# facebookresearch/metamorph

Hardware: AMD Instinct MI355X
Metric: train tokens/sec (LLaMA-3-8B + SigLIP-SO400M, seq2048, 256 img toks), whole job (higher is better)
Workload: dtype bf16

## Files before the change

include/mm355.h:

```cpp
#ifndef MM355_H
#define MM355_H

#include <stddef.h>
#include <stdint.h>

#ifdef __cplusplus
extern "C" {
#endif

#define MM355_VERSION 100

#define MM355_OK            0
#define MM355_EINVAL       -1
#define MM355_EUNSUPPORTED -2
#define MM355_ELAUNCH      -3

typedef uint16_t mm355_bf16;

int mm355_version(void);
const char* mm355_strerror(int code);

#define MM355_GEMM_BIAS        1u
#define MM355_GEMM_GELU_ERF    2u
#define MM355_GEMM_GELU_TANH   4u
// ... 17 lines not shown
int64_t mm355_gemm_splitk_swiglu_ws_floats(int64_t M, int64_t I, int64_t K);
int mm355_gemm_splitk_swiglu_bf16(const mm355_bf16* X, int64_t ldx, const mm355_bf16* Wgu, int64_t ldw, mm355_bf16* act, int64_t ld_act,
                                  int64_t M, int64_t I, int64_t K, float* workspace, int64_t workspace_floats, void* stream);
int mm355_gemm_splitk_rope_append_bf16(const mm355_bf16* X, int64_t ldx, const mm355_bf16* Wqkv, int64_t ldw, mm355_bf16* qkv, int64_t ld_qkv,
                                       int64_t M, int64_t Hq, int64_t Hkv, int64_t d, int64_t K, const mm355_bf16* cos_t,
                                       const mm355_bf16* sin_t, const int32_t* positions, mm355_bf16* k_cache, mm355_bf16* v_cache,
                                       int64_t ld_kv, int64_t batch_stride_kv, float* workspace, int64_t workspace_floats, void* stream);

int mm355_gemm_swiglu_bf16(const mm355_bf16* X, int64_t ldx, const mm355_bf16* Wgu, int64_t ldw, mm355_bf16* gu, int64_t ld_gu,
                           mm355_bf16* act, int64_t ld_act, int64_t M, int64_t I, int64_t K, void* stream);

int mm355_gemm_rope_bf16(const mm355_bf16* X, int64_t ldx, const mm355_bf16* Wqkv, int64_t ldw, mm355_bf16* qkv, int64_t ld_qkv,
                         const mm355_bf16* cos_t, const mm355_bf16* sin_t, const int32_t* pos_offset,
                         int64_t M, int64_t N, int64_t K, int64_t L, int64_t n_rot, void* stream);

int mm355_gemm_swiglu_bwd_bf16(const mm355_bf16* dY, int64_t ldy, const mm355_bf16* WdT, int64_t ldw, const mm355_bf16* gu, int64_t ld_gu,
                               mm355_bf16* dgu, int64_t ld_dgu, mm355_bf16* actT, mm355_bf16* dguT, int64_t ldT,
                               int64_t M, int64_t I, int64_t K, void* stream);

int mm355_gemm_pair_bf16(const mm355_bf16* A0, int64_t lda0, const mm355_bf16* B0, int64_t ldb0, void* C0, int64_t ldc0,
                         int64_t M0, int64_t N0, int64_t K0, uint32_t flags0,
                         const mm355_bf16* A1, int64_t lda1, const mm355_bf16* B1, int64_t ldb1, void* C1, int64_t ldc1,
                         int64_t M1, int64_t N1, int64_t K1, uint32_t flags1, void* stream);

int mm355_transpose_bf16(const mm355_bf16* in, int64_t ld_in, int64_t rows, int64_t cols,
                         mm355_bf16* out, int64_t ld_out, void* stream);

int mm355_colsum_bf16(const mm355_bf16* dY, int64_t ld, int64_t M, int64_t N, float* db_f32, void* stream);

int mm355_rmsnorm_fwd(const mm355_bf16* x, const mm355_bf16* w, mm355_bf16* y, int64_t M, int64_t h,
                      float eps, void* stream);
int mm355_rmsnorm_fwd_rstd(const mm355_bf16* x, const mm355_bf16* w, mm355_bf16* y, float* rstd_out, int64_t M, int64_t h,
                           float eps, void* stream);
int mm355_rmsnorm_apply_t(const mm355_bf16* x, const mm355_bf16* w, const float* rstd, int64_t M, int64_t h,
                          mm355_bf16* out_t, int64_t ld_out, void* stream);
int mm355_rmsnorm_bwd(const mm355_bf16* dy, const mm355_bf16* x, const mm355_bf16* w,
                      const mm355_bf16* dres, mm355_bf16* dx, float* dw_f32, float* workspace,
                      int64_t M, int64_t h, float eps, void* stream);
int64_t mm355_rmsnorm_bwd_ws_floats(int64_t M, int64_t h);
int mm355_rmsnorm_bwd_wgrad(const mm355_bf16* dy, const mm355_bf16* x, const mm355_bf16* w, const mm355_bf16* dres,
                            mm355_bf16* dx, mm355_bf16* w_grad, int accumulate, float* workspace,
                            int64_t M, int64_t h, float eps, void* stream);

int mm355_layernorm_fwd(const mm355_bf16* x, const mm355_bf16* w, const mm355_bf16* b, mm355_bf16* y,
                        int64_t M, int64_t h, float eps, void* stream);
int64_t mm355_layernorm_bwd_ws_floats(int64_t M, int64_t h);
// ... 178 lines not shown
                     int64_t n_seg, mm355_bf16* dembed, int64_t h, int accumulate, void* stream);

int mm355_im2col_patch(const void* images, int images_are_f32, int64_t N, int64_t H, int64_t W, int64_t p,
                       mm355_bf16* out, int64_t Kp, void* stream);
int mm355_bilinear_l2norm(const mm355_bf16* in, mm355_bf16* out, int64_t N, int64_t side_in, int64_t side_out,
                          int64_t C, int normalize, void* stream);
int mm355_bilinear_l2norm_bwd(const mm355_bf16* in, const mm355_bf16* d_out, float* d_in_f32, int64_t N, int64_t side_in,
                              int64_t side_out, int64_t C, int normalize, void* stream);

int mm355_cosine_loss(const mm355_bf16* pred_raw, const mm355_bf16* target, int64_t R, int64_t C, int normalize,
                      float* cos_sum, mm355_bf16* dpred, float* row_ws, void* stream);

int mm355_mean_abs_loss(const mm355_bf16* pred, const mm355_bf16* target, int64_t R, int64_t C, float* abs_sum,
                        mm355_bf16* dpred, float* row_ws, void* stream);
int mm355_soft_ce_loss(const mm355_bf16* pred_raw, const mm355_bf16* target, int64_t R, int64_t C, int normalize,
                       float temperature, float* loss_sum, mm355_bf16* dpred, float* row_ws, void* stream);
int mm355_softmax_rows(const mm355_bf16* x, mm355_bf16* y, int64_t R, int64_t C, float temperature, void* stream);
int mm355_softmax_rows_bwd(const mm355_bf16* y, const mm355_bf16* dy, mm355_bf16* dx, int64_t R, int64_t C,
                           float temperature, void* stream);

int mm355_adamw_shard(float* p32, float* m, float* v, const mm355_bf16* g, mm355_bf16* p_out, int64_t n,
                      float lr, float beta1, float beta2, float eps, float weight_decay,
                      float bias_corr1, float bias_corr2, const float* grad_scale_dev, void* stream);
#define MM355_SUMSQ_PARTIALS 2048
int mm355_sumsq_bf16(const mm355_bf16* x, int64_t n, float* out, float* partials, void* stream);
int mm355_clip_coef(const float* sumsq, float max_norm, float pre_scale, float* coef, void* stream);

#ifdef __cplusplus
}
#endif
#endif
```

metamorph_amd/csrc/elementwise.hip:

```cpp
#include "mm355_common.h"
#include <algorithm>

namespace {

constexpr int NT = 256;
constexpr int MAX_GRID = 256 * 16;

inline unsigned grid_for(int64_t work_items) {
    int64_t g = (work_items + NT - 1) / NT;
    if (g > MAX_GRID) g = MAX_GRID;
    if (g < 1) g = 1;
    return (unsigned)g;
}

__global__ void rope_table_kernel(uint16_t* __restrict__ cos_o, uint16_t* __restrict__ sin_o, int L, int d, float theta) {
    const int half = d >> 1;
    for (int64_t i = blockIdx.x * (int64_t)NT + threadIdx.x; i < (int64_t)L * half; i += (int64_t)gridDim.x * NT) {
        const int l = (int)(i / half), j = (int)(i % half);
        const float inv = 1.0f / powf(theta, (float)(2 * j) / (float)d);
        const float ang = (float)l * inv;
        const uint16_t c = f2bf(cosf(ang)), s = f2bf(sinf(ang));
        cos_o[(int64_t)l * d + j] = c; cos_o[(int64_t)l * d + half + j] = c;
        sin_o[(int64_t)l * d + j] = s; sin_o[(int64_t)l * d + half + j] = s;
    }
}

__global__ void rope_table_freq_kernel(uint16_t* __restrict__ cos_o, uint16_t* __restrict__ sin_o, int L, int d,
                                       const float* __restrict__ inv_freq, float scaling) {
    const int half = d >> 1;
// ... 150 lines not shown
template <typename TX>
__global__ __launch_bounds__(NT) void axpy_kernel(uint16_t* __restrict__ y, const TX* __restrict__ x, int64_t n, const float* __restrict__ s_dev,
                                                  float s_host, int accumulate) {
    const float s = (s_dev ? *s_dev : 1.0f) * s_host;
    for (int64_t i = blockIdx.x * (int64_t)NT + threadIdx.x; i < n; i += (int64_t)gridDim.x * NT) {
        float xv;
        if constexpr (sizeof(TX) == 2) xv = bf2f(x[i]); else xv = x[i];
        float r = s * xv;
        if (accumulate) r += bf2f(y[i]);
        y[i] = f2bf(r);
    }
}
__global__ __launch_bounds__(NT) void cast2d_kernel(const float* __restrict__ in, int64_t ld_in, uint16_t* __restrict__ out, int64_t ld_out, int64_t rows, int cols) {
    const int cv = cols >> 3;
    const int64_t total = rows * cv;
    for (int64_t i = blockIdx.x * (int64_t)NT + threadIdx.x; i < total; i += (int64_t)gridDim.x * NT) {
        const int64_t r = i / cv; const int c = (int)(i % cv) * 8;
        const f32x4 a = *(const f32x4*)(in + r * ld_in + c), b = *(const f32x4*)(in + r * ld_in + c + 4);
        const float f[8] = {a.x, a.y, a.z, a.w, b.x, b.y, b.z, b.w};
        *(u32x4*)(out + r * ld_out + c) = pack8(f);
    }
}

__global__ __launch_bounds__(NT) void adamw_kernel(float* __restrict__ p32, float* __restrict__ m, float* __restrict__ v, const uint16_t* __restrict__ g,
                                                   uint16_t* __restrict__ pout, int64_t n, float lr, float b1, float b2, float eps, float wd,
                                                   float bc1, float bc2, const float* __restrict__ gs_dev) {
    const float gs = gs_dev ? *gs_dev : 1.0f;
    const float inv_sqrt_bc2 = rsqrtf(bc2);
    const float step = lr / bc1;
    for (int64_t i = blockIdx.x * (int64_t)NT + threadIdx.x; i < n; i += (int64_t)gridDim.x * NT) {
        const float gr = bf2f(g[i]) * gs;
        float p = p32[i] * (1.0f - lr * wd);
        const float mi = m[i] * b1 + (1.0f - b1) * gr;
        const float vi = v[i] * b2 + (1.0f - b2) * gr * gr;
        const float denom = sqrtf(vi) * inv_sqrt_bc2 + eps;
        p -= step * (mi / denom);
        m[i] = mi; v[i] = vi; p32[i] = p;
        pout[i] = f2bf(p);
    }
}
__global__ __launch_bounds__(NT) void sumsq_kernel(const uint16_t* __restrict__ x, int64_t n, float* __restrict__ partials) {
    __shared__ float red[NT / 64];
    float s = 0.f;
    const int64_t nv = n >> 3;
    for (int64_t v = blockIdx.x * (int64_t)NT + threadIdx.x; v < nv; v += (int64_t)gridDim.x * NT) {
        float f[8];
        unpack8(*(const u32x4*)(x + v * 8), f);
#pragma unroll
        for (int e = 0; e < 8; ++e) s += f[e] * f[e];
    }
    if (blockIdx.x == 0 && threadIdx.x < (n & 7)) { const float f = bf2f(x[(nv << 3) + threadIdx.x]); s += f * f; }
    s = block_sum<NT>(s, red);
    if (threadIdx.x == 0) partials[blockIdx.x] = s;
}
__global__ __launch_bounds__(NT) void sumsq_finish_kernel(const float* __restrict__ partials, int count, float* __restrict__ out) {
    __shared__ float red[NT / 64];
    float s = 0.f;
    for (int i = threadIdx.x; i < count; i += NT) s += partials[i];
    s = block_sum<NT>(s, red);
// ... 158 lines not shown
    if (!x || n <= 0 || !mm_aligned16(x)) return MM355_EINVAL;
    LAUNCH(scale_kernel, grid_for(n / 8 + 1), x, n, s_dev, s_host);
}
extern "C" int mm355_axpy_bf16(mm355_bf16* y, const mm355_bf16* x, int64_t n, const float* s_dev, float s_host, int accumulate, void* stream) {
    (void)hipGetLastError();
    if (!x || !y || n <= 0) return MM355_EINVAL;
    LAUNCH(axpy_kernel<uint16_t>, grid_for(n), y, x, n, s_dev, s_host, accumulate);
}
extern "C" int mm355_axpy_f32_to_bf16(mm355_bf16* y, const float* x, int64_t n, float s_host, int accumulate, void* stream) {
    (void)hipGetLastError();
    if (!x || !y || n <= 0) return MM355_EINVAL;
    LAUNCH(axpy_kernel<float>, grid_for(n), y, x, n, (const float*)nullptr, s_host, accumulate);
}
extern "C" int mm355_axpy_f32_to_bf16_dev(mm355_bf16* y, const float* x, int64_t n, const float* s_dev, float s_host, int accumulate, void* stream) {
    (void)hipGetLastError();
    if (!x || !y || n <= 0) return MM355_EINVAL;
    LAUNCH(axpy_kernel<float>, grid_for(n), y, x, n, s_dev, s_host, accumulate);
}
extern "C" int mm355_cast_f32_bf16_2d(const float* in, int64_t ld_in, mm355_bf16* out, int64_t ld_out, int64_t rows, int64_t cols, void* stream) {
    (void)hipGetLastError();
    if (!in || !out || rows <= 0 || cols <= 0 || (cols & 7) || (ld_in & 3) || (ld_out & 7)) return MM355_EINVAL;
    LAUNCH(cast2d_kernel, grid_for(rows * (cols / 8)), in, ld_in, out, ld_out, rows, (int)cols);
}
extern "C" int mm355_adamw_shard(float* p32, float* m, float* v, const mm355_bf16* g, mm355_bf16* p_out, int64_t n, float lr, float beta1,
                                 float beta2, float eps, float weight_decay, float bias_corr1, float bias_corr2, const float* grad_scale_dev,
                                 void* stream) {
    (void)hipGetLastError();
    if (!p32 || !m || !v || !g || !p_out || n <= 0 || bias_corr1 <= 0.f || bias_corr2 <= 0.f) return MM355_EINVAL;
    LAUNCH(adamw_kernel, grid_for(n), p32, m, v, g, p_out, n, lr, beta1, beta2, eps, weight_decay, bias_corr1, bias_corr2, grad_scale_dev);
}
extern "C" int mm355_sumsq_bf16(const mm355_bf16* x, int64_t n, float* out, float* partials, void* stream) {
    (void)hipGetLastError();
    if (!x || !out || !partials || n <= 0 || !mm_aligned16(x)) return MM355_EINVAL;
    const int blocks = (int)std::min<int64_t>((n / 8 + NT) / NT, MM355_SUMSQ_PARTIALS);
    hipLaunchKernelGGL(sumsq_kernel, dim3(blocks), dim3(NT), 0, (hipStream_t)stream, x, n, partials);
    hipLaunchKernelGGL(sumsq_finish_kernel, dim3(1), dim3(NT), 0, (hipStream_t)stream, (const float*)partials, blocks, out);
    return mm_launch_status();
}
extern "C" int mm355_clip_coef(const float* sumsq, float max_norm, float pre_scale, float* coef, void* stream) {
    (void)hipGetLastError();
    if (!sumsq || !coef) return MM355_EINVAL;
    hipLaunchKernelGGL(clip_coef_kernel, dim3(1), dim3(1), 0, (hipStream_t)stream, sumsq, max_norm, pre_scale, coef);
    return mm_launch_status();
}
extern "C" int mm355_im2col_patch(const void* images, int images_are_f32, int64_t N, int64_t H, int64_t W, int64_t p, mm355_bf16* out, int64_t Kp,
                                  void* stream) {
    (void)hipGetLastError();
    if (!images || !out || N <= 0 || H < p || W < p || p <= 0 || Kp < 3 * p * p) return MM355_EINVAL;
    const int64_t total = N * (H / p) * (W / p) * Kp;
    if (images_are_f32) LAUNCH(im2col_kernel<float>, grid_for(total), (const float*)images, (int)N, (int)H, (int)W, (int)p, out, (int)Kp);
    LAUNCH(im2col_kernel<uint16_t>, grid_for(total), (const uint16_t*)images, (int)N, (int)H, (int)W, (int)p, out, (int)Kp);
}
// ... 25 lines not shown
```

metamorph_amd/csrc/gemm_bf16.hip:

```cpp
#include "gemm_common.h"
#include "splitk.h"
#include <type_traits>
#include <cstdlib>

namespace {

MM_DEV void gemm_epilogue_swiglu(f32x4 (&acc)[8][4], const GemmArgs& a, unsigned char* smem, int m0, int tn, int wm, int wn, int wave, int lane) {
    constexpr int TN = 64;
    const int fr = lane & 15, fq = lane >> 4;
    const int M = a.M, I = (int)a.res_mod;
    float* stg = (float*)smem + wave * (16 * TN);
    const int row_l = lane >> 2, k4 = lane & 3;
    uint16_t* gu = (uint16_t*)a.C;
    uint16_t* act = (uint16_t*)a.res;
    const int ch0 = tn * 128 + wn * 32;
#pragma unroll
    for (int i = 0; i < 8; ++i) {
        __builtin_amdgcn_fence(__ATOMIC_RELEASE, "wavefront");
        __builtin_amdgcn_wave_barrier();
#pragma unroll
        for (int j = 0; j < 4; ++j)
#pragma unroll
            for (int r = 0; r < 4; ++r) stg[(fq * 4 + r) * TN + j * 16 + fr] = acc[i][j][r];
        __builtin_amdgcn_fence(__ATOMIC_RELEASE, "wavefront");
// ... 638 lines not shown
}

template <int ABL = 0>
__global__ __launch_bounds__(512) void gemm_pp_kernel(GemmArgs a) {
    extern __shared__ __attribute__((aligned(16))) unsigned char smem[];
#ifdef MM355_PP_PERSIST
    const int total = a.ntm * a.ntn;
    for (int bid = blockIdx.x; bid < total; bid += gridDim.x) {
        gemm_pp_tile<ABL>(a, bid, smem);
        __syncthreads();
    }
#else
    gemm_pp_tile<ABL>(a, blockIdx.x, smem);
#endif
}

__global__ __launch_bounds__(512) void gemm_pp_pair_kernel(GemmArgs a0, GemmArgs a1, int n0) {
    extern __shared__ __attribute__((aligned(16))) unsigned char smem[];
    const int bid = blockIdx.x;
    if (bid < n0) gemm_pp_tile(a0, bid, smem);
    else gemm_pp_tile(a1, bid - n0, smem);
}

template <int BM, int BN, int WM, int WN, bool GLDS, int PIPE>
int launch_gemm(GemmArgs a, hipStream_t s);

constexpr int PP_LDS = 2 * (256 + 256) * 128;

int64_t pp_prepare(GemmArgs& a) {
    a.ntm = (a.M + 255) / 256;
    a.ntn = (a.N + 255) / 256;
    a.gm = 4;
    return (int64_t)a.ntm * a.ntn;
}

template <int ABL = 0>
int launch_gemm_pp_t(GemmArgs a, hipStream_t s) {
    static std::atomic<uint64_t> lds_ok{0};
    if (mm_ensure_dynamic_lds((const void*)gemm_pp_kernel<ABL>, PP_LDS, lds_ok) != MM355_OK) return MM355_ELAUNCH;
    const int64_t total = pp_prepare(a);
    if (total <= 0 || total > 0x7fffffff) return MM355_EINVAL;
#ifdef MM355_PP_PERSIST
    hipLaunchKernelGGL((gemm_pp_kernel<ABL>), dim3((unsigned)std::min<int64_t>(total, MM355_PP_PERSIST)), dim3(512), PP_LDS, s, a);
#else
    hipLaunchKernelGGL((gemm_pp_kernel<ABL>), dim3((unsigned)total), dim3(512), PP_LDS, s, a);
#endif
    return mm_launch_status();
}

int launch_gemm_pp_pair(GemmArgs a0, GemmArgs a1, hipStream_t s) {
    static std::atomic<uint64_t> lds_ok{0};
    if (mm_ensure_dynamic_lds((const void*)gemm_pp_pair_kernel, PP_LDS, lds_ok) != MM355_OK) return MM355_ELAUNCH;
    const int64_t n0 = pp_prepare(a0), n1 = pp_prepare(a1);
    if (n0 <= 0 || n1 <= 0 || n0 + n1 > 0x7fffffff) return MM355_EINVAL;
    hipLaunchKernelGGL(gemm_pp_pair_kernel, dim3((unsigned)(n0 + n1)), dim3(512), PP_LDS, s, a0, a1, (int)n0);
    return mm_launch_status();
}

bool pp_eligible(const GemmArgs& a) {
    if (a.K < 128 || (a.K & 127)) return false;
    const int64_t ea = (256 * a.lda + a.K) * 2;
    const int64_t eb = (256 * a.ldb + a.K) * 2;
    return ea < 0x7fffffffLL && eb < 0x7fffffffLL;
}

int launch_gemm_pp(GemmArgs a, hipStream_t s) {
    if (!pp_eligible(a)) return launch_gemm<256, 256, 2, 4, true, 1>(a, s);
    return launch_gemm_pp_t(a, s);
}

template <int BM, int BN, int WM, int WN, bool GLDS, int PIPE = 0>
int launch_gemm(GemmArgs a, hipStream_t s) {
    constexpr int STAGE = (BM + BN) * 128;
    constexpr int LDS = 2 * STAGE;
    auto kern = gemm_nt_kernel<BM, BN, WM, WN, GLDS, PIPE>;
    static std::atomic<uint64_t> lds_ok{0};
    if (mm_ensure_dynamic_lds((const void*)kern, LDS, lds_ok) != MM355_OK) return MM355_ELAUNCH;
    a.ntm = (a.M + BM - 1) / BM;
// ... 422 lines not shown
    if (!dma_ok && variant != 1) return MM355_EUNSUPPORTED;
    switch (variant) {
        case 1: return launch_gemm<128, 128, 2, 2, false>(a, s);
        case 2: return launch_gemm<128, 128, 2, 2, true>(a, s);
        case 7: return launch_gemm<256, 256, 2, 4, true, 1>(a, s);
        case 9: return launch_gemm<64, 128, 1, 4, true>(a, s);
        case 11: return launch_gemm_pp(a, s);
#ifdef MM355_ABLATIONS
        case 91: return launch_gemm_pp_t<1>(a, s);
        case 92: return launch_gemm_pp_t<2>(a, s);
        case 93: return launch_gemm_pp_t<3>(a, s);
#endif
        default: return MM355_EUNSUPPORTED;
    }
}

namespace {
int pair_problem(GemmArgs& a, const mm355_bf16* A, int64_t lda, const mm355_bf16* B, int64_t ldb, void* C, int64_t ldc,
                 int64_t M, int64_t N, int64_t K, uint32_t flags) {
    if (!A || !B || !C || M <= 0 || N <= 0 || K <= 0) return MM355_EINVAL;
    if ((K & 7) || (lda & 7) || (ldb & 7) || !mm_aligned16(A) || !mm_aligned16(B) || !mm_aligned16(C)) return MM355_EINVAL;
    if (M > 0x7fffffff || N > 0x7fffffff || K > 0x7fffffff) return MM355_EINVAL;
    if (flags & ~(MM355_GEMM_ACCUMULATE | MM355_GEMM_OUT_F32)) return MM355_EINVAL;
    a.A = A; a.B = B; a.C = C; a.bias = nullptr; a.res = nullptr;
    a.lda = lda; a.ldb = ldb; a.ldc = ldc; a.ldr = 0; a.res_mod = 0;
    a.M = (int)M; a.N = (int)N; a.K = (int)K; a.flags = flags; a.ntm = a.ntn = 0;
    return pp_eligible(a) ? MM355_OK : MM355_EUNSUPPORTED;
}
}

extern "C" int mm355_gemm_pair_bf16(const mm355_bf16* A0, int64_t lda0, const mm355_bf16* B0, int64_t ldb0, void* C0, int64_t ldc0,
                                    int64_t M0, int64_t N0, int64_t K0, uint32_t flags0,
                                    const mm355_bf16* A1, int64_t lda1, const mm355_bf16* B1, int64_t ldb1, void* C1, int64_t ldc1,
                                    int64_t M1, int64_t N1, int64_t K1, uint32_t flags1, void* stream) {
    (void)hipGetLastError();
    GemmArgs a0, a1;
    int rc = pair_problem(a0, A0, lda0, B0, ldb0, C0, ldc0, M0, N0, K0, flags0);
    if (rc != MM355_OK) return rc;
    rc = pair_problem(a1, A1, lda1, B1, ldb1, C1, ldc1, M1, N1, K1, flags1);
    if (rc != MM355_OK) return rc;
    return launch_gemm_pp_pair(a0, a1, (hipStream_t)stream);
}

extern "C" int mm355_transpose_bf16(const mm355_bf16* in, int64_t ld_in, int64_t rows, int64_t cols, mm355_bf16* out,
                                    int64_t ld_out, void* stream) {
    (void)hipGetLastError();
    if (!in || !out || rows <= 0 || cols <= 0 || (ld_in & 7) || !mm_aligned16(in) || !mm_aligned16(out)) return MM355_EINVAL;
    if (ld_out < rows || rows > 0x7fffffff || cols > 0x7fffffff) return MM355_EINVAL;
    dim3 grid((unsigned)((cols + 63) / 64), (unsigned)((rows + 63) / 64));
    hipLaunchKernelGGL(transpose_kernel, grid, dim3(256), 0, (hipStream_t)stream, in, ld_in, (int)rows, (int)cols, out, ld_out);
    return mm_launch_status();
}

extern "C" int mm355_gemm_swiglu_bf16(const mm355_bf16* X, int64_t ldx, const mm355_bf16* Wgu, int64_t ldw, mm355_bf16* gu, int64_t ld_gu,
                                      mm355_bf16* act, int64_t ld_act, int64_t M, int64_t I, int64_t K, void* stream) {
    (void)hipGetLastError();
    if (!X || !Wgu || !gu || !act || M <= 0 || I <= 0 || K <= 0) return MM355_EINVAL;
    if ((ldx & 7) || (ldw & 7) || (ld_gu & 7) || (ld_act & 7) || !mm_aligned16(X) || !mm_aligned16(Wgu) || !mm_aligned16(gu) || !mm_aligned16(act))
        return MM355_EINVAL;
    if (M > 0x7fffffff || I > 0x3fffffff || K > 0x7fffffff) return MM355_EINVAL;
    if ((I & 127) || K < 128 || (K & 127) || (2 * I * ldw + K) * 2 >= 0x7fffffffLL || (256 * ldx + K) * 2 >= 0x7fffffffLL) return MM355_EUNSUPPORTED;
    GemmArgs a = {};
    a.A = X; a.B = Wgu; a.C = gu; a.bias = nullptr; a.res = act;
    a.lda = ldx; a.ldb = ldw; a.ldc = ld_gu; a.ldr = ld_act; a.res_mod = I;
// ... 65 lines not shown
```

metamorph_amd/functional.py:

```python
from __future__ import annotations

import os

import numpy as np
import torch
from torch.autograd import Function

from . import ops

BF16 = torch.bfloat16
VARIANTS = {"fuse_swiglu": True, "fuse_rope": True, "fuse_swiglu_bwd": True, "decode_graph": True, "decode_fused": True,
            "wt_cache": False,
            "decode_fold_rows": 4,
            "prefill_splitk": True,
            "decode_wide_fused": True, "decode_wide_gu_gemv": True,
            "prefill_fused": True,
            "w8_gemm": True,
            "extend_pass": True, "extend_min_rows": 3}


def set_variant(name, value):
    if name not in VARIANTS:
        raise KeyError(f"unknown variant {name!r}: {sorted(VARIANTS)}")
    old, VARIANTS[name] = VARIANTS[name], (int(value) if isinstance(VARIANTS[name], int) and not isinstance(VARIANTS[name], bool) else bool(value))
    return old


_CUS = 256



def _adjacent(ts):
    t0 = ts[0]
    ptr = t0.data_ptr()
    st = t0.untyped_storage()
    total = sum(t.numel() * t.element_size() for t in ts)
    if ptr - st.data_ptr() + total > st.nbytes():
        return False
    for t in ts:
        if (not t.is_contiguous() or t.data_ptr() != ptr or t.shape[1:] != t0.shape[1:] or t.dtype != t0.dtype
                or t.untyped_storage().data_ptr() != st.data_ptr()):
# ... 150 lines not shown
def transposed_weight(w, sources=None):
    if sources is None or not VARIANTS["wt_cache"]:
        return transpose_padded(w)
    key = (w.untyped_storage().data_ptr(), w.storage_offset(), tuple(w.shape), tuple(w.stride()))
    stamp = (param_generation(),) + tuple(p._version for p in sources)
    hit = _WT_CACHE.get(key)
    if hit is not None and hit[0] == stamp:
        return hit[1]
    if _WT_CACHE and next(iter(_WT_CACHE.values()))[0][0] != stamp[0]:
        _WT_CACHE.clear()
    wt = transpose_padded(w)
    _WT_CACHE[key] = (stamp, wt)
    return wt


def drop_transposed_weights():
    _WT_CACHE.clear()


def _pairable(a0, b0, a1, b1):
    t0 = -(-a0.shape[0] // 256) * -(-b0.shape[0] // 256)
    t1 = -(-a1.shape[0] // 256) * -(-b1.shape[0] // 256)
    return min(t0, t1) >= 200 and t0 % 8 == 0 and ops.gemm_pair_supported(a0, b0, a1, b1)


def input_grad_gemm(dy2d, w, out=None, residual=None):
    return ops.gemm(dy2d, transposed_weight(w), out=out, residual=residual)



class LayerMeta:

    def __init__(self, B, L, Hq, Hkv, d, I, eps, cos, sin, seqlens, recompute=False, pos_offset=None, c2p=None, p2c=None):
        self.B, self.L, self.Hq, self.Hkv, self.d, self.I, self.eps = B, L, Hq, Hkv, d, I, eps
        self.cos, self.sin, self.seqlens = cos, sin, seqlens
        self.pos_offset = pos_offset
        self.c2p, self.p2c = c2p, p2c
        self.prompt_pass = False
        self.scale = d ** -0.5
        self.recompute = recompute


PROMPT_GU_SPLITK_ROWS = 64


def decoder_layer_forward(x, layer, m: LayerMeta):
# ... 127 lines not shown
                do = torch.empty((dx2.shape[0], woT.shape[0]), device=dev, dtype=BF16)
                ops.gemm_pair(a0, b0, buf, acc, dx2, woT, do, False)
            else:
                do = ops.gemm(dx2, woT)
                ops.gemm(a0, b0, out=buf, accumulate=acc)
            del a0, b0, woT
            commit_grad(att.o_proj.weight, buf)
        if do is None:
            do = input_grad_gemm(dx2, att.o_proj.weight)
        dqkv = torch.empty_like(qkv)
        fuse_rope = VARIANTS["fuse_rope"] and ops.attn_bwd_rope_supported(m.d)
        o_att = o
        if m.p2c is not None:
            o_att, do = ops.rows_gather(o, m.p2c), ops.rows_gather(do, m.p2c)
        ops.attn_bwd(qkv[:, :nq], qkv[:, nq:nq + nk], qkv[:, nq + nk:], o_att, do, lse, m.B, m.L, m.Hq, m.Hkv, m.d,
                     m.scale, True, m.seqlens, dqkv[:, :nq], dqkv[:, nq:nq + nk], dqkv[:, nq + nk:],
                     rope=(m.cos, m.sin, m.pos_offset) if fuse_rope else None)
        del do, o_att
        if not fuse_rope:
            ops.rope_qk_(dqkv, m.B, m.L, m.Hq, m.Hkv, m.d, m.cos, m.sin, inverse=True, pos_offset=m.pos_offset)
        if m.c2p is not None:
            dqkv = ops.rows_gather(dqkv, m.c2p)
        wqkv = fused_weight(qkv_params)
        dn1 = ops.gemm(dqkv, transposed_weight(wqkv, sources=qkv_params))
        if any(p.requires_grad for p in qkv_params):
            fb, acc, bufs = fused_grad_target(qkv_params)
            n1T = ops.rmsnorm_apply_t(x, layer.input_layernorm.weight, rstd1, _padded_rows(x.shape[0], long_k=True))
            if held is not None:
                a1, b1 = _dw_operands(dqkv, None, xT=n1T)
                if ops.gemm_pair_supported(held[0], held[1], a1, b1):
                    ops.gemm_pair(held[0], held[1], held[2], held[3], a1, b1, fb, bool(acc))
                else:
                    ops.gemm(held[0], held[1], out=held[2], accumulate=held[3])
                    ops.gemm(a1, b1, out=fb, accumulate=bool(acc))
                held = None
                del a1, b1
            else:
                weight_grad_gemm(dqkv, None, fb, bool(acc), xT=n1T)
            commit_fused_grad(qkv_params, fb, acc, bufs)
            del n1T
        del dqkv
        dx = _rmsnorm_backward(dn1, x, layer.input_layernorm.weight, m.eps, dx2)
        if _LAYER_GRAD_HOOK is not None:
            _LAYER_GRAD_HOOK(layer)
        return (dx, None, None) + (None,) * (len(ctx.needs_input_grad) - 3)


def decoder_layer(x, layer, meta):
    params_ready(layer)
    ws = [p for p in layer.parameters()]
    if torch.is_grad_enabled() and (x.requires_grad or any(p.requires_grad for p in ws)):
        return DecoderLayerFn.apply(x, layer, meta, *ws)
    return decoder_layer_forward(x, layer, meta)[0]



class RmsNormFn(Function):
    @staticmethod
    def forward(ctx, x, w, eps):
        ctx.save_for_backward(x, w)
        ctx.eps = eps
        return ops.rmsnorm_fwd(x, w.data if isinstance(w, torch.nn.Parameter) else w, eps)

# ... 1052 lines not shown
```

metamorph_amd/ops.py:

```python
from __future__ import annotations

import os

import torch

from . import lib as _lib

BF16 = torch.bfloat16

GEMM_BIAS, GEMM_GELU_ERF, GEMM_GELU_TANH, GEMM_RESIDUAL, GEMM_ACCUMULATE, GEMM_OUT_F32 = 1, 2, 4, 8, 16, 32
GELU_ERF, GELU_TANH = 0, 1


def _L():
    return _lib.load()


def _stream():
    return torch.cuda.current_stream().cuda_stream


def _chk_dev(*ts):
    for t in ts:
        if t is not None and not t.is_cuda:
# ... 128 lines not shown
def gemm_pair_supported(a0, b0, a1, b1):
    return (a0.shape[1] == b0.shape[1] and a1.shape[1] == b1.shape[1]
            and gemm_pp_operands_ok(a0.shape[1], a0, b0) and gemm_pp_operands_ok(a1.shape[1], a1, b1))


def gemm_pair(a0, b0, out0, acc0, a1, b1, out1, acc1):
    _chk_dev(a0, b0, out0, a1, b1, out1)
    probs = []
    for a, b, out, acc in ((a0, b0, out0, acc0), (a1, b1, out1, acc1)):
        assert a.dtype == BF16 and b.dtype == BF16
        pa, M, K, lda = _rows2d(a)
        pb, N, Kb, ldb = _rows2d(b)
        assert K == Kb, (a.shape, b.shape)
        po, Mo, No, ldc = _rows2d(out)
        assert (Mo, No) == (M, N), (out.shape, M, N)
        assert out.dtype in (BF16, torch.float32)
        flags = (GEMM_ACCUMULATE if acc else 0) | (GEMM_OUT_F32 if out.dtype == torch.float32 else 0)
        probs += [pa, lda, pb, ldb, po, ldc, M, N, K, flags]
    _lib.check(_L().mm355_gemm_pair_bf16(*probs, _stream()),
               f"mm355_gemm_pair_bf16 {tuple(a0.shape)}x{tuple(b0.shape)} + {tuple(a1.shape)}x{tuple(b1.shape)}")
    return out0, out1


def gemm_pp_operands_ok(K, *mats):
    return K >= 128 and K % 128 == 0 and all(256 * m.stride(0) * 2 < 2 ** 31 - 2 ** 20 for m in mats)


def gemv_supported(x, w):
    _, M, K, ldx = _rows2d(x)
    _, N, _, ldw = _rows2d(w)
    if M > 32 or (M > 16 and not gemv_rows32_units((N + 3) // 4)):
        return False
    return M <= 4 or ((N - 1) * ldw * 2 + K * 2 < 0xf0000000 and (M - 1) * ldx * 2 + K * 2 < 0xf0000000)


def gemv_rows32_units(units):
    return (units + 3) // 4 > 1280


def gemv(x, w, out=None, bias=None, residual=None, gelu=None):
    _chk_dev(x, w, out, bias, residual)
    px, M, K, ldx = _rows2d(x)
    pw, N, Kw, ldw = _rows2d(w)
    assert K == Kw and x.dtype == BF16 and w.dtype == BF16
    if out is None:
        out = torch.empty((M, N), device=x.device, dtype=BF16)
# ... 905 lines not shown
def bilinear_l2norm(feat, side_in, side_out, normalize):
    _chk_dev(feat)
    assert feat.is_contiguous()
    N, P, C = feat.shape
    assert P == side_in * side_in
    out = torch.empty((N, side_out * side_out, C), device=feat.device, dtype=BF16)
    _lib.check(_L().mm355_bilinear_l2norm(feat.data_ptr(), out.data_ptr(), N, side_in, side_out, C, int(normalize), _stream()), "mm355_bilinear_l2norm")
    return out


def bilinear_l2norm_bwd(x, dy, side_in, side_out, normalize):
    _chk_dev(x, dy)
    assert x.is_contiguous() and dy.is_contiguous()
    N, _, C = x.shape
    acc = torch.zeros(x.shape, device=x.device, dtype=torch.float32)
    _lib.check(_L().mm355_bilinear_l2norm_bwd(x.data_ptr(), dy.data_ptr(), acc.data_ptr(), N, side_in, side_out, C, int(bool(normalize)),
                                              _stream()), "mm355_bilinear_l2norm_bwd")
    out = torch.empty_like(x)
    cast_f32_to_bf16_2d(acc.view(-1, C), out.view(-1, C))
    return out



def adamw_shard_(p32, m, v, g, p_out, lr, beta1, beta2, eps, wd, step, grad_scale_dev=None):
    _chk_dev(p32, m, v, g, p_out)
    n = p32.numel()
    assert m.numel() == n and v.numel() == n and g.numel() == n and p_out.numel() == n
    bc1 = 1.0 - beta1 ** step
    bc2 = 1.0 - beta2 ** step
    _lib.check(_L().mm355_adamw_shard(p32.data_ptr(), m.data_ptr(), v.data_ptr(), g.data_ptr(), p_out.data_ptr(), n, lr, beta1, beta2,
                                      eps, wd, bc1, bc2, _p(grad_scale_dev), _stream()), "mm355_adamw_shard")


SUMSQ_PARTIALS = 2048
_sumsq_partials = {}


def sumsq_(x, out_f32, partials=None):
    _chk_dev(x, out_f32)
    assert x.is_contiguous()
    if partials is None:
        key = (x.device, _stream())
        partials = _sumsq_partials.get(key)
        if partials is None:
            partials = _sumsq_partials[key] = torch.empty(SUMSQ_PARTIALS, dtype=torch.float32, device=x.device)
    assert partials.dtype == torch.float32 and partials.numel() >= SUMSQ_PARTIALS and partials.device == x.device
    _lib.check(_L().mm355_sumsq_bf16(x.data_ptr(), x.numel(), out_f32.data_ptr(), partials.data_ptr(), _stream()), "mm355_sumsq_bf16")
    return out_f32


def clip_coef(sumsq_f32, max_norm, pre_scale, out_f32):
    _chk_dev(sumsq_f32, out_f32)
    _lib.check(_L().mm355_clip_coef(sumsq_f32.data_ptr(), max_norm, pre_scale, out_f32.data_ptr(), _stream()), "mm355_clip_coef")
    return out_f32
# ... 1 lines not shown
```

Before: 26610.

## Group QKV input-grad and weight-grad GEMMs into one launch; vectorize AdamW

```diff
diff --git a/include/mm355.h b/include/mm355.h
--- a/include/mm355.h
+++ b/include/mm355.h
@@ -63,6 +63,17 @@
                          int64_t M0, int64_t N0, int64_t K0, uint32_t flags0,
                          const mm355_bf16* A1, int64_t lda1, const mm355_bf16* B1, int64_t ldb1, void* C1, int64_t ldc1,
                          int64_t M1, int64_t N1, int64_t K1, uint32_t flags1, void* stream);
+
+#define MM355_GEMM_GROUP_MAX 4
+typedef struct mm355_gemm_problem {
+    const mm355_bf16* A; int64_t lda;
+    const mm355_bf16* B; int64_t ldb;
+    void* C; int64_t ldc;
+    const mm355_bf16* residual; int64_t ldr;
+    int64_t M, N, K;
+    uint32_t flags;
+} mm355_gemm_problem;
+int mm355_gemm_group_bf16(const mm355_gemm_problem* problems, int count, void* stream);
 
 int mm355_transpose_bf16(const mm355_bf16* in, int64_t ld_in, int64_t rows, int64_t cols,
                          mm355_bf16* out, int64_t ld_out, void* stream);
@@ -287,6 +298,9 @@
 int mm355_adamw_shard(float* p32, float* m, float* v, const mm355_bf16* g, mm355_bf16* p_out, int64_t n,
                       float lr, float beta1, float beta2, float eps, float weight_decay,
                       float bias_corr1, float bias_corr2, const float* grad_scale_dev, void* stream);
+int mm355_adamw_shard_opt(float* p32, float* m, float* v, const mm355_bf16* g, mm355_bf16* p_out, int64_t n,
+                          float lr, float beta1, float beta2, float eps, float weight_decay,
+                          float bias_corr1, float bias_corr2, const float* grad_scale_dev, int kernel, int grid, void* stream);
 #define MM355_SUMSQ_PARTIALS 2048
 int mm355_sumsq_bf16(const mm355_bf16* x, int64_t n, float* out, float* partials, void* stream);
 int mm355_clip_coef(const float* sumsq, float max_norm, float pre_scale, float* coef, void* stream);
diff --git a/metamorph_amd/csrc/elementwise.hip b/metamorph_amd/csrc/elementwise.hip
--- a/metamorph_amd/csrc/elementwise.hip
+++ b/metamorph_amd/csrc/elementwise.hip
@@ -5,6 +5,7 @@
 
 constexpr int NT = 256;
 constexpr int MAX_GRID = 256 * 16;
+constexpr int ADAMW8_GRID = 256 * 8;
 
 inline unsigned grid_for(int64_t work_items) {
     int64_t g = (work_items + NT - 1) / NT;
@@ -201,6 +202,14 @@
     }
 }
 
+MM_DEV void adamw_elem(float& p, float& mi, float& vi, const float gr, const float lr, const float b1, const float b2, const float eps, const float wd,
+                       const float inv_sqrt_bc2, const float step) {
+    p = p * (1.0f - lr * wd);
+    mi = mi * b1 + (1.0f - b1) * gr;
+    vi = vi * b2 + (1.0f - b2) * gr * gr;
+    const float denom = sqrtf(vi) * inv_sqrt_bc2 + eps;
+    p -= step * (mi / denom);
+}
 __global__ __launch_bounds__(NT) void adamw_kernel(float* __restrict__ p32, float* __restrict__ m, float* __restrict__ v, const uint16_t* __restrict__ g,
                                                    uint16_t* __restrict__ pout, int64_t n, float lr, float b1, float b2, float eps, float wd,
                                                    float bc1, float bc2, const float* __restrict__ gs_dev) {
@@ -209,11 +218,40 @@
     const float step = lr / bc1;
     for (int64_t i = blockIdx.x * (int64_t)NT + threadIdx.x; i < n; i += (int64_t)gridDim.x * NT) {
         const float gr = bf2f(g[i]) * gs;
-        float p = p32[i] * (1.0f - lr * wd);
-        const float mi = m[i] * b1 + (1.0f - b1) * gr;
-        const float vi = v[i] * b2 + (1.0f - b2) * gr * gr;
-        const float denom = sqrtf(vi) * inv_sqrt_bc2 + eps;
-        p -= step * (mi / denom);
+        float p = p32[i], mi = m[i], vi = v[i];
+        adamw_elem(p, mi, vi, gr, lr, b1, b2, eps, wd, inv_sqrt_bc2, step);
+        m[i] = mi; v[i] = vi; p32[i] = p;
+        pout[i] = f2bf(p);
+    }
+}
+__global__ __launch_bounds__(NT) void adamw8_kernel(float* __restrict__ p32, float* __restrict__ m, float* __restrict__ v, const uint16_t* __restrict__ g,
+                                                    uint16_t* __restrict__ pout, int64_t n, float lr, float b1, float b2, float eps, float wd,
+                                                    float bc1, float bc2, const float* __restrict__ gs_dev) {
+    const float gs = gs_dev ? *gs_dev : 1.0f;
+    const float inv_sqrt_bc2 = rsqrtf(bc2);
+    const float step = lr / bc1;
+    const int64_t nv = n >> 3;
+    for (int64_t i = blockIdx.x * (int64_t)NT + threadIdx.x; i < nv; i += (int64_t)gridDim.x * NT) {
+        const int64_t e0 = i << 3;
+        const f32x4 pa = *(const f32x4*)(p32 + e0), pb = *(const f32x4*)(p32 + e0 + 4);
+        const f32x4 ma = *(const f32x4*)(m + e0), mb = *(const f32x4*)(m + e0 + 4);
+        const f32x4 va = *(const f32x4*)(v + e0), vb = *(const f32x4*)(v + e0 + 4);
+        float p[8] = {pa.x, pa.y, pa.z, pa.w, pb.x, pb.y, pb.z, pb.w};
+        float mi[8] = {ma.x, ma.y, ma.z, ma.w, mb.x, mb.y, mb.z, mb.w};
+        float vi[8] = {va.x, va.y, va.z, va.w, vb.x, vb.y, vb.z, vb.w};
+        float gr[8];
+        unpack8(*(const u32x4*)(g + e0), gr);
+#pragma unroll
+        for (int e = 0; e < 8; ++e) adamw_elem(p[e], mi[e], vi[e], gr[e] * gs, lr, b1, b2, eps, wd, inv_sqrt_bc2, step);
+        *(f32x4*)(m + e0) = f32x4{mi[0], mi[1], mi[2], mi[3]}; *(f32x4*)(m + e0 + 4) = f32x4{mi[4], mi[5], mi[6], mi[7]};
+        *(f32x4*)(v + e0) = f32x4{vi[0], vi[1], vi[2], vi[3]}; *(f32x4*)(v + e0 + 4) = f32x4{vi[4], vi[5], vi[6], vi[7]};
+        *(f32x4*)(p32 + e0) = f32x4{p[0], p[1], p[2], p[3]}; *(f32x4*)(p32 + e0 + 4) = f32x4{p[4], p[5], p[6], p[7]};
+        *(u32x4*)(pout + e0) = pack8(p);
+    }
+    if (blockIdx.x == 0 && threadIdx.x < (n & 7)) {
+        const int64_t i = (nv << 3) + threadIdx.x;
+        float p = p32[i], mi = m[i], vi = v[i];
+        adamw_elem(p, mi, vi, bf2f(g[i]) * gs, lr, b1, b2, eps, wd, inv_sqrt_bc2, step);
         m[i] = mi; v[i] = vi; p32[i] = p;
         pout[i] = f2bf(p);
     }
@@ -418,12 +456,26 @@
     if (!in || !out || rows <= 0 || cols <= 0 || (cols & 7) || (ld_in & 3) || (ld_out & 7)) return MM355_EINVAL;
     LAUNCH(cast2d_kernel, grid_for(rows * (cols / 8)), in, ld_in, out, ld_out, rows, (int)cols);
 }
+extern "C" int mm355_adamw_shard_opt(float* p32, float* m, float* v, const mm355_bf16* g, mm355_bf16* p_out, int64_t n, float lr, float beta1,
+                                     float beta2, float eps, float weight_decay, float bias_corr1, float bias_corr2, const float* grad_scale_dev,
+                                     int kernel, int grid, void* stream) {
+    (void)hipGetLastError();
+    if (!p32 || !m || !v || !g || !p_out || n <= 0 || bias_corr1 <= 0.f || bias_corr2 <= 0.f) return MM355_EINVAL;
+    if (kernel < 0 || kernel > 2 || grid < 0 || grid > 65536) return MM355_EINVAL;
+    const bool aligned = mm_aligned16(p32) && mm_aligned16(m) && mm_aligned16(v) && mm_aligned16(g) && mm_aligned16(p_out);
+    if (kernel == 2 && !aligned) return MM355_EINVAL;
+    if (kernel == 1 || !aligned) {
+        LAUNCH(adamw_kernel, grid ? (unsigned)grid : grid_for(n), p32, m, v, g, p_out, n, lr, beta1, beta2, eps, weight_decay, bias_corr1, bias_corr2,
+               grad_scale_dev);
+    }
+    unsigned blocks = grid ? (unsigned)grid : (unsigned)std::min<int64_t>((n / 8 + NT - 1) / NT, ADAMW8_GRID);
+    if (blocks < 1) blocks = 1;
+    LAUNCH(adamw8_kernel, blocks, p32, m, v, g, p_out, n, lr, beta1, beta2, eps, weight_decay, bias_corr1, bias_corr2, grad_scale_dev);
+}
 extern "C" int mm355_adamw_shard(float* p32, float* m, float* v, const mm355_bf16* g, mm355_bf16* p_out, int64_t n, float lr, float beta1,
                                  float beta2, float eps, float weight_decay, float bias_corr1, float bias_corr2, const float* grad_scale_dev,
                                  void* stream) {
-    (void)hipGetLastError();
-    if (!p32 || !m || !v || !g || !p_out || n <= 0 || bias_corr1 <= 0.f || bias_corr2 <= 0.f) return MM355_EINVAL;
-    LAUNCH(adamw_kernel, grid_for(n), p32, m, v, g, p_out, n, lr, beta1, beta2, eps, weight_decay, bias_corr1, bias_corr2, grad_scale_dev);
+    return mm355_adamw_shard_opt(p32, m, v, g, p_out, n, lr, beta1, beta2, eps, weight_decay, bias_corr1, bias_corr2, grad_scale_dev, 0, 0, stream);
 }
 extern "C" int mm355_sumsq_bf16(const mm355_bf16* x, int64_t n, float* out, float* partials, void* stream) {
     (void)hipGetLastError();
diff --git a/metamorph_amd/csrc/gemm_bf16.hip b/metamorph_amd/csrc/gemm_bf16.hip
--- a/metamorph_amd/csrc/gemm_bf16.hip
+++ b/metamorph_amd/csrc/gemm_bf16.hip
@@ -684,6 +684,19 @@
     else gemm_pp_tile(a1, bid - n0, smem);
 }
 
+struct GemmGroup {
+    GemmArgs a[MM355_GEMM_GROUP_MAX];
+    int end[MM355_GEMM_GROUP_MAX];
+};
+__global__ __launch_bounds__(512) void gemm_pp_group_kernel(GemmGroup g) {
+    extern __shared__ __attribute__((aligned(16))) unsigned char smem[];
+    static_assert(MM355_GEMM_GROUP_MAX == 4, "the pick below counts three boundaries");
+    const int bid = blockIdx.x;
+    const int pi = (bid >= g.end[0]) + (bid >= g.end[1]) + (bid >= g.end[2]);
+    const int first = pi ? g.end[pi - 1] : 0;
+    gemm_pp_tile(g.a[pi], bid - first, smem);
+}
+
 template <int BM, int BN, int WM, int WN, bool GLDS, int PIPE>
 int launch_gemm(GemmArgs a, hipStream_t s);
 
@@ -716,6 +729,24 @@
     const int64_t n0 = pp_prepare(a0), n1 = pp_prepare(a1);
     if (n0 <= 0 || n1 <= 0 || n0 + n1 > 0x7fffffff) return MM355_EINVAL;
     hipLaunchKernelGGL(gemm_pp_pair_kernel, dim3((unsigned)(n0 + n1)), dim3(512), PP_LDS, s, a0, a1, (int)n0);
+    return mm_launch_status();
+}
+
+int launch_gemm_pp_group(GemmGroup& g, int count, hipStream_t s) {
+    static std::atomic<uint64_t> lds_ok{0};
+    if (mm_ensure_dynamic_lds((const void*)gemm_pp_group_kernel, PP_LDS, lds_ok) != MM355_OK) return MM355_ELAUNCH;
+    int64_t total = 0;
+    for (int i = 0; i < MM355_GEMM_GROUP_MAX; ++i) {
+        if (i < count) {
+            const int64_t n = pp_prepare(g.a[i]);
+            if (n <= 0) return MM355_EINVAL;
+            if (i + 1 < count && (n & 7)) return MM355_EUNSUPPORTED;
+            total += n;
+            if (total > 0x7fffffff) return MM355_EINVAL;
+        } else g.a[i] = g.a[0];
+        g.end[i] = (int)total;
+    }
+    hipLaunchKernelGGL(gemm_pp_group_kernel, dim3((unsigned)total), dim3(512), PP_LDS, s, g);
     return mm_launch_status();
 }
 
@@ -1184,9 +1215,10 @@
     if ((K & 7) || (lda & 7) || (ldb & 7) || !mm_aligned16(A) || !mm_aligned16(B) || !mm_aligned16(C)) return MM355_EINVAL;
     if (M > 0x7fffffff || N > 0x7fffffff || K > 0x7fffffff) return MM355_EINVAL;
     if (flags & ~(MM355_GEMM_ACCUMULATE | MM355_GEMM_OUT_F32)) return MM355_EINVAL;
-    a.A = A; a.B = B; a.C = C; a.bias = nullptr; a.res = nullptr;
-    a.lda = lda; a.ldb = ldb; a.ldc = ldc; a.ldr = 0; a.res_mod = 0;
-    a.M = (int)M; a.N = (int)N; a.K = (int)K; a.flags = flags; a.ntm = a.ntn = 0;
+    a = GemmArgs{};
+    a.A = A; a.B = B; a.C = C;
+    a.lda = lda; a.ldb = ldb; a.ldc = ldc;
+    a.M = (int)M; a.N = (int)N; a.K = (int)K; a.flags = flags;
     return pp_eligible(a) ? MM355_OK : MM355_EUNSUPPORTED;
 }
 }
@@ -1202,6 +1234,28 @@
     rc = pair_problem(a1, A1, lda1, B1, ldb1, C1, ldc1, M1, N1, K1, flags1);
     if (rc != MM355_OK) return rc;
     return launch_gemm_pp_pair(a0, a1, (hipStream_t)stream);
+}
+
+extern "C" int mm355_gemm_group_bf16(const mm355_gemm_problem* problems, int count, void* stream) {
+    (void)hipGetLastError();
+    if (!problems || count < 1 || count > MM355_GEMM_GROUP_MAX) return MM355_EINVAL;
+    int order[MM355_GEMM_GROUP_MAX];
+    for (int i = 0; i < count; ++i) {
+        int j = i;
+        for (; j > 0 && problems[order[j - 1]].K < problems[i].K; --j) order[j] = order[j - 1];
+        order[j] = i;
+    }
+    GemmGroup g;
+    for (int i = 0; i < count; ++i) {
+        const mm355_gemm_problem& p = problems[order[i]];
+        if (p.flags & ~(MM355_GEMM_ACCUMULATE | MM355_GEMM_OUT_F32 | MM355_GEMM_RESIDUAL)) return MM355_EINVAL;
+        if ((p.flags & MM355_GEMM_RESIDUAL) && (!p.residual || !mm_aligned16(p.residual))) return MM355_EINVAL;
+        const int rc = pair_problem(g.a[i], p.A, p.lda, p.B, p.ldb, p.C, p.ldc, p.M, p.N, p.K, p.flags & ~MM355_GEMM_RESIDUAL);
+        if (rc != MM355_OK) return rc;
+        g.a[i].flags = p.flags;
+        if (p.flags & MM355_GEMM_RESIDUAL) { g.a[i].res = p.residual; g.a[i].ldr = p.ldr; }
+    }
+    return launch_gemm_pp_group(g, count, (hipStream_t)stream);
 }
 
 extern "C" int mm355_transpose_bf16(const mm355_bf16* in, int64_t ld_in, int64_t rows, int64_t cols, mm355_bf16* out,
diff --git a/metamorph_amd/functional.py b/metamorph_amd/functional.py
--- a/metamorph_amd/functional.py
+++ b/metamorph_amd/functional.py
@@ -16,7 +16,8 @@
             "decode_wide_fused": True, "decode_wide_gu_gemv": True,
             "prefill_fused": True,
             "w8_gemm": True,
-            "extend_pass": True, "extend_min_rows": 3}
+            "extend_pass": True, "extend_min_rows": 3,
+            "gemm_group": True}
 
 
 def set_variant(name, value):
@@ -213,6 +214,11 @@
     t0 = -(-a0.shape[0] // 256) * -(-b0.shape[0] // 256)
     t1 = -(-a1.shape[0] // 256) * -(-b1.shape[0] // 256)
     return min(t0, t1) >= 200 and t0 % 8 == 0 and ops.gemm_pair_supported(a0, b0, a1, b1)
+
+
+def _groupable(problems):
+    return (all(-(-p[0].shape[0] // 256) * -(-p[1].shape[0] // 256) >= 200 for p in problems)
+            and ops.gemm_group_supported([(p[0], p[1], None, False) for p in problems]))
 
 
 def input_grad_gemm(dy2d, w, out=None, residual=None):
@@ -386,23 +392,32 @@
         if m.c2p is not None:
             dqkv = ops.rows_gather(dqkv, m.c2p)
         wqkv = fused_weight(qkv_params)
-        dn1 = ops.gemm(dqkv, transposed_weight(wqkv, sources=qkv_params))
+        wqkvT = transposed_weight(wqkv, sources=qkv_params)
+        dn1 = None
         if any(p.requires_grad for p in qkv_params):
             fb, acc, bufs = fused_grad_target(qkv_params)
             n1T = ops.rmsnorm_apply_t(x, layer.input_layernorm.weight, rstd1, _padded_rows(x.shape[0], long_k=True))
-            if held is not None:
-                a1, b1 = _dw_operands(dqkv, None, xT=n1T)
-                if ops.gemm_pair_supported(held[0], held[1], a1, b1):
+            a1, b1 = _dw_operands(dqkv, None, xT=n1T)
+            group = ([held[:4]] if held is not None else []) + [(a1, b1, fb, bool(acc))]
+            if VARIANTS["gemm_group"] and _groupable(group + [(dqkv, wqkvT)]):
+                dn1 = torch.empty((dqkv.shape[0], wqkvT.shape[0]), device=dev, dtype=BF16)
+                ops.gemm_group(group + [(dqkv, wqkvT, dn1, False)])
+            else:
+                dn1 = ops.gemm(dqkv, wqkvT)
+                if held is None:
+                    ops.gemm(a1, b1, out=fb, accumulate=bool(acc))
+                elif ops.gemm_pair_supported(held[0], held[1], a1, b1):
                     ops.gemm_pair(held[0], held[1], held[2], held[3], a1, b1, fb, bool(acc))
                 else:
                     ops.gemm(held[0], held[1], out=held[2], accumulate=held[3])
                     ops.gemm(a1, b1, out=fb, accumulate=bool(acc))
-                held = None
-                del a1, b1
-            else:
-                weight_grad_gemm(dqkv, None, fb, bool(acc), xT=n1T)
+            held = None
+            del a1, b1, group
             commit_fused_grad(qkv_params, fb, acc, bufs)
             del n1T
+        if dn1 is None:
+            dn1 = ops.gemm(dqkv, wqkvT)
+        del wqkvT
         del dqkv
         dx = _rmsnorm_backward(dn1, x, layer.input_layernorm.weight, m.eps, dx2)
         if _LAYER_GRAD_HOOK is not None:
diff --git a/metamorph_amd/ops.py b/metamorph_amd/ops.py
--- a/metamorph_amd/ops.py
+++ b/metamorph_amd/ops.py
@@ -1,5 +1,6 @@
 from __future__ import annotations
 
+import ctypes
 import os
 
 import torch
@@ -174,6 +175,52 @@
     return out0, out1
 
 
+GEMM_GROUP_MAX = 4
+
+
+class _GemmProblem(ctypes.Structure):
+    _fields_ = [("A", ctypes.c_void_p), ("lda", ctypes.c_int64), ("B", ctypes.c_void_p), ("ldb", ctypes.c_int64),
+                ("C", ctypes.c_void_p), ("ldc", ctypes.c_int64), ("residual", ctypes.c_void_p), ("ldr", ctypes.c_int64),
+                ("M", ctypes.c_int64), ("N", ctypes.c_int64), ("K", ctypes.c_int64), ("flags", ctypes.c_uint32)]
+
+
+def _group_problem(p):
+    a, b, out, acc = p[:4]
+    return a, b, out, acc, (p[4] if len(p) > 4 else None)
+
+
+def gemm_group_supported(problems):
+    if not 1 <= len(problems) <= GEMM_GROUP_MAX:
+        return False
+    tiles = []
+    for a, b, out, acc, res in map(_group_problem, problems):
+        if a.shape[1] != b.shape[1] or not gemm_pp_operands_ok(a.shape[1], a, b):
+            return False
+        tiles.append((-a.shape[1], len(tiles), -(-a.shape[0] // 256) * -(-b.shape[0] // 256)))
+    return all(t % 8 == 0 for _, _, t in sorted(tiles)[:-1])
+
+
+def gemm_group(problems):
+    arr = (_GemmProblem * len(problems))()
+    what = []
+    for q, (a, b, out, acc, res) in zip(arr, map(_group_problem, problems)):
+        _chk_dev(a, b, out, res)
+        assert a.dtype == BF16 and b.dtype == BF16 and out.dtype in (BF16, torch.float32)
+        q.A, q.M, q.K, q.lda = _rows2d(a)
+        q.B, q.N, Kb, q.ldb = _rows2d(b)
+        assert q.K == Kb, (a.shape, b.shape)
+        q.C, Mo, No, q.ldc = _rows2d(out)
+        assert (Mo, No) == (q.M, q.N), (out.shape, q.M, q.N)
+        q.flags = (GEMM_ACCUMULATE if acc else 0) | (GEMM_OUT_F32 if out.dtype == torch.float32 else 0)
+        if res is not None:
+            assert res.dtype == BF16 and tuple(res.shape) == (q.M, q.N)
+            q.residual, _, _, q.ldr = _rows2d(res)
+            q.flags |= GEMM_RESIDUAL
+        what.append(f"{tuple(a.shape)}x{tuple(b.shape)}")
+    _lib.check(_L().mm355_gemm_group_bf16(ctypes.addressof(arr), len(problems), _stream()), "mm355_gemm_group_bf16 " + " + ".join(what))
+    return [p[2] for p in problems]
+
+
 def gemm_pp_operands_ok(K, *mats):
     return K >= 128 and K % 128 == 0 and all(256 * m.stride(0) * 2 < 2 ** 31 - 2 ** 20 for m in mats)
 
@@ -1125,14 +1172,14 @@
 
 
 
-def adamw_shard_(p32, m, v, g, p_out, lr, beta1, beta2, eps, wd, step, grad_scale_dev=None):
+def adamw_shard_(p32, m, v, g, p_out, lr, beta1, beta2, eps, wd, step, grad_scale_dev=None, *, kernel=0, grid=0):
     _chk_dev(p32, m, v, g, p_out)
     n = p32.numel()
     assert m.numel() == n and v.numel() == n and g.numel() == n and p_out.numel() == n
     bc1 = 1.0 - beta1 ** step
     bc2 = 1.0 - beta2 ** step
-    _lib.check(_L().mm355_adamw_shard(p32.data_ptr(), m.data_ptr(), v.data_ptr(), g.data_ptr(), p_out.data_ptr(), n, lr, beta1, beta2,
-                                      eps, wd, bc1, bc2, _p(grad_scale_dev), _stream()), "mm355_adamw_shard")
+    _lib.check(_L().mm355_adamw_shard_opt(p32.data_ptr(), m.data_ptr(), v.data_ptr(), g.data_ptr(), p_out.data_ptr(), n, lr, beta1, beta2,
+                                          eps, wd, bc1, bc2, _p(grad_scale_dev), kernel, grid, _stream()), "mm355_adamw_shard")
 
 
 SUMSQ_PARTIALS = 2048
```

After: 26520. No clear change (-0.3%).
